# danielbrathwaite/OpenGL-Path-Tracing

Hardware: AMD Instinct MI355X
Metric: Mrays/sec + ms/frame @1920×1080, 8 bounces, 1/2/4/8 MI355X (higher is better)
Workload: dtype f32

## Files before the change

opengl-path-tracing_amd/csrc/pt_pool.h:

```cpp
#pragma once

#include <stdint.h>

#include "pt_math.h"

namespace ptpool {

constexpr int kLanes = 64;
constexpr int kMaxPaths = 128;
constexpr int kRecDwords = 20;
constexpr int kChunks = kRecDwords / 4;

enum : int { kChunkO = 0, kChunkD = 1, kChunkInc = 2, kChunkCol = 3, kChunkItem = 4 };

PT_HD int quad_of(int c, int i, int P) { return c * P + i; }
PT_HD int list_bytes(int P) { return (P + 15) & ~15; }
PT_HD int wave_bytes(int P) { return P * kRecDwords * 4 + list_bytes(P); }

constexpr uint32_t kNoItem = 0xffffffffu;
PT_HD bool pack_ok(int width, int rows_local, int n_frames, int max_bounce, int n_slots, int n_spheres) {
    return width >= 1 && width <= 65535 && rows_local >= 0 && rows_local <= 65535 && n_frames >= 1 &&
           n_frames <= 65535 && max_bounce >= 0 && max_bounce <= 65533 && n_slots >= 0 && n_slots <= 65533 &&
           n_spheres == 1 && (long long)n_frames * (long long)(max_bounce + 2) < (1ll << 31);
}
PT_HD uint32_t pack_xy(int lx, int crow) { return (uint32_t)lx | ((uint32_t)crow << 16); }
PT_HD int xy_lx(uint32_t v) { return (int)(v & 0xffffu); }
PT_HD int xy_crow(uint32_t v) { return (int)(v >> 16); }
PT_HD uint32_t pack_k(int k, int kend) { return (uint32_t)k | ((uint32_t)kend << 16); }
PT_HD int k_k(uint32_t v) { return (int)(v & 0xffffu); }
PT_HD int k_kend(uint32_t v) { return (int)(v >> 16); }
PT_HD uint32_t pack_hit(int hprim, int bounce) { return (uint32_t)(hprim + 2) | ((uint32_t)(bounce + 1) << 16); }
PT_HD int hit_hprim(uint32_t v) { return (int)(v & 0xffffu) - 2; }
PT_HD int hit_bounce(uint32_t v) { return (int)(v >> 16) - 1; }
PT_HD uint32_t with_hprim(uint32_t v, int hprim) { return (v & 0xffff0000u) | (uint32_t)(hprim + 2); }
PT_HD uint32_t pack_cost(uint32_t pcost, bool report) { return pcost | (report ? 0x80000000u : 0u); }
PT_HD uint32_t cost_of(uint32_t v) { return v & 0x7fffffffu; }
PT_HD bool cost_report(uint32_t v) { return (v >> 31) != 0u; }

enum : int { kShade = 0, kLeaf = 1 };
struct Lists { int nS, nL; };

PT_HD int choose(const Lists& l) { return l.nS >= l.nL ? kShade : kLeaf; }
PT_HD int take(const Lists& l, int phase) {
    const int n = phase == kShade ? l.nS : l.nL;
    return n < kLanes ? n : kLanes;
}
PT_HD int pop_index(const Lists& l, int phase, int n, int lane, int P) {
    return phase == kShade ? l.nS - n + lane : P - l.nL + lane;
}
PT_HD void drop(Lists& l, int phase, int n) {
    if (phase == kShade) l.nS -= n; else l.nL -= n;
}
PT_HD int push_index(const Lists& l, int phase, int rank, int P) {
    return phase == kShade ? l.nS + rank : P - 1 - l.nL - rank;
}
PT_HD void grow(Lists& l, int phase, int n) {
    if (phase == kShade) l.nS += n; else l.nL += n;
}

PT_HD size_t block_bytes(int P, int waves, size_t scene_bytes) {
    return ((scene_bytes + 15) & ~(size_t)15) + (size_t)waves * (size_t)wave_bytes(P);
}

}
```

opengl-path-tracing_amd/csrc/pt_render_pool.h:

```cpp
#ifndef PT_POOL_SWEEP_DEPTH
#define PT_POOL_SWEEP_DEPTH 2
#endif
#ifndef PT_POOL_SWEEP_LDS
#define PT_POOL_SWEEP_LDS 1
#endif
#ifndef PT_POOL_SWEEP_SIGNED
#define PT_POOL_SWEEP_SIGNED 1
#endif
#define PT_POOL_SIGNED_ON (PT_POOL_SWEEP_SIGNED && PT_POOL_SWEEP_LDS && PT_POOL_SWEEP_DEPTH > 0)
namespace {

__device__ __forceinline__ void pool_cold_walk(const KParams& p, const SceneView& S, f3 o, f3 d, float& t, int& hprim) {
    int w = 0;
    while (w >= 0) {
        const float4 lo = p.sc.nodes[2 * w], hi = p.sc.nodes[2 * w + 1];
        const int a = __float_as_int(hi.z), b = __float_as_int(hi.w);
        if (!slab(lo, hi, o, d, t)) { w = b; continue; }
        if (a >= 0) { w = a; continue; }
        const int q = (~a) >> 2;
        const int s0 = 2 * __float_as_int(p.sweep_tab[2 * q + 1].w);
        const bool cop = __float_as_int(tri_quad<true>(S, s0 + 1, 1).w) != 0;
        const float4 nda = tri_quad<true>(S, s0, 0);
        const float4 ndb = cop ? nda : tri_quad<true>(S, s0 + 1, 0);
        const float ta = tri_plane(nda, o, d);
        const float tb = cop ? ta : tri_plane(ndb, o, d);
        bool oka = false, okb = false, ca = false, cb = false;
        if (win_open(ta, t)) oka = tri_edges_at<true, false>(S, s0, mk(nda.x, nda.y, nda.z), o + d * ta, false, 0.0f, ca);
        if (win_closed(tb, t)) okb = tri_edges_at<true, false>(S, s0 + 1, mk(ndb.x, ndb.y, ndb.z), o + d * tb, false, 0.0f, cb);
        const float h1 = oka ? ta : -1.0f, h2 = okb ? tb : -1.0f;
        const LeafChoice lc = leaf_choice(h1, h2, t);
        if (lc.c1 | lc.c2) {
            t = lc.c1 ? h1 : h2;
            hprim = s0 + (lc.c1 ? 0 : 1);
        }
        w = b;
    }
}

__device__ __forceinline__ void pool_pass_fence() {
    __builtin_amdgcn_fence(__ATOMIC_RELEASE, "wavefront");
    __builtin_amdgcn_wave_barrier();
    __builtin_amdgcn_fence(__ATOMIC_ACQUIRE, "wavefront");
}

template <int NT, int P, int MINW>
__global__ __launch_bounds__(NT, MINW) void k_render_pool(KParams p) {
    static_assert(P >= 64 && P <= ptpool::kMaxPaths && P % 4 == 0, "one-byte list entries in a 16-byte padded array");
    using namespace ptpool;
    const LaunchFacts<true, true> F{p};
    const const_v4f* const sweep_tab = (const const_v4f*)(size_t)p.sweep_tab;
    (void)sweep_tab;
    resolve_frames(p);
    extern __shared__ float4 lds[];
    const int T = p.n_slots, nt = 4 * T, nm = 3 * p.n_mats, ns = 2, nb = ptc::kSignedQuads * p.n_sweep;
    stage_tris_chain_order(lds, p, T, NT);
    for (int i = threadIdx.x; i < nm; i += NT) lds[nt + i] = p.sc.mats[i];
    for (int i = threadIdx.x; i < ns; i += NT) lds[nt + nm + i] = p.sc.spheres[i];
#if PT_POOL_SIGNED_ON
    for (int leaf = threadIdx.x; leaf < p.n_sweep; leaf += NT) {
        const float4 a = p.sweep_tab[2 * leaf], b = p.sweep_tab[2 * leaf + 1];
        for (int axis = 0; axis < ptc::kSignedQuads; axis++) {
            float q[4];
            ptc::sweep_signed_quad(a, b, axis, q);
            lds[nt + nm + ns + ptc::kSignedQuads * leaf + axis] = make_float4(q[0], q[1], q[2], q[3]);
        }
    }
#else
    for (int i = threadIdx.x; i < 2 * p.n_sweep; i += NT) lds[nt + nm + ns + i] = p.sweep_tab[i];
#endif
    const int scene_q = nt + nm + ns + nb;
    const int lane = (int)(threadIdx.x & 63u);
    float4* const pool = lds + scene_q + (int)(threadIdx.x >> 6) * (wave_bytes(P) / 16);
    unsigned char* const list = (unsigned char*)(pool + kChunks * P);
    for (int i = lane; i < P; i += kLanes) {
        pool[quad_of(kChunkO, i, P)] = make_float4(0, 0, 0, -1.0f);
        pool[quad_of(kChunkD, i, P)] = make_float4(0, 0, 1, 0);
        pool[quad_of(kChunkInc, i, P)] = make_float4(0, 0, 0, __uint_as_float(pack_hit(-1, -1)));
        pool[quad_of(kChunkCol, i, P)] = make_float4(1, 1, 1, 0);
        pool[quad_of(kChunkItem, i, P)] = make_float4(__uint_as_float(kNoItem), 0, 0, 0);
        list[i] = (unsigned char)i;
    }
    __syncthreads();
    SceneView S;
    S.nodes = nullptr;
    S.tris = lds;
    S.mats = lds + nt;
    S.spheres = lds + nt + nm;
    const float4* const boxes = lds + nt + nm + ns;
    const float2* const signed_pairs = (const float2*)boxes;
    (void)signed_pairs;
    S.np = 0;
    S.tp = T;
    S.cm[0] = p.cons_m[0], S.cm[1] = p.cons_m[1], S.cm[2] = p.cons_m[2];
    S.ws[0] = p.win_slack[0], S.ws[1] = p.win_slack[1], S.ws[2] = p.win_slack[2];
    S.clo = ptc::kWindowLo;
    const f3 cpos = mk(p.cam[0], p.cam[1], p.cam[2]), cfwd = mk(p.cam[3], p.cam[4], p.cam[5]);
    const f3 cright = mk(p.cam[6], p.cam[7], p.cam[8]), cup = mk(p.cam[9], p.cam[10], p.cam[11]);
    const int tiles_x = (p.W + 7) >> 3;
    const unsigned n_groups = (unsigned)((p.n_frames + p.group - 1) / p.group);
    const unsigned total_ids = p.queue_tiles * n_groups * 64u;
    unsigned qnext = 0, qend = 0;
    Lists L = {P, 0};
    while (L.nS + L.nL > 0) {
        const int phase = choose(L), n = take(L, phase);
        const bool on = lane < n;
        int idx = 0;
        if (on) idx = list[pop_index(L, phase, n, lane, P)];
        drop(L, phase, n);
        bool to_shade = false, to_leaf = false;
        if (phase == kShade) {
            const float4 c0 = pool[quad_of(kChunkO, idx, P)], c1 = pool[quad_of(kChunkD, idx, P)];
            const float4 c2 = pool[quad_of(kChunkInc, idx, P)], c3 = pool[quad_of(kChunkCol, idx, P)];
            const float4 c4 = pool[quad_of(kChunkItem, idx, P)];
            f3 o = mk(c0.x, c0.y, c0.z), d = mk(c1.x, c1.y, c1.z), inc = mk(c2.x, c2.y, c2.z), col = mk(c3.x, c3.y, c3.z);
            float t = c0.w;
            unsigned bi = __float_as_uint(c1.w);
            int hprim = hit_hprim(__float_as_uint(c2.w)), bounce = hit_bounce(__float_as_uint(c2.w));
            uint32_t state = __float_as_uint(c3.w);
            unsigned xy = __float_as_uint(c4.x);
            int aidx = __float_as_int(c4.y);
            int k = k_k(__float_as_uint(c4.z)), kend = k_kend(__float_as_uint(c4.z));
            unsigned pcost = cost_of(__float_as_uint(c4.w));
            bool report = cost_report(__float_as_uint(c4.w));
            bool retired = false;
            if (on && !(t < 0.0f)) {
                const bool hit = hprim != -1;
                pcost++;
                f3 rgb;
                const bool finished = shade_segment<true>(F, p, S, hit, hprim, t, o, d, inc, col, state, bounce, rgb);
                if (finished) {
                    bounce = -1;
                    const f3 px = (mk(0, 0, 0) + rgb) / 1.0f;
                    nt_store3(p.rgb + 3 * ((size_t)k * (size_t)(p.rows_local * p.W) + (size_t)aidx), px);
                    k++;
                }
                t = -1.0f;
            }
            if (on & (bounce < 0) & (xy != kNoItem) & (k >= kend)) {
                if (report) atomicAdd(&p.tile_cost[(xy_crow(xy) >> 3) * tiles_x + (xy_lx(xy) >> 3)], pcost);
                xy = kNoItem;
            }
            const bool want = on && xy == kNoItem;
            const unsigned long long m = __ballot(want);
            if (m) {
                const QueueIds qi = queue_ids<true>(p, want, m, qnext, qend);
                const unsigned id = qi.id;
                qnext = qi.qnext, qend = qi.qend;
                if (want) {
                    if (id >= total_ids) {
                        retired = true;
                    } else {
                        const unsigned item = id >> 6, w = id & 63u;
                        const unsigned tile = p.grp_magic ? __umulhi(item, p.grp_magic) : item;
                        const int g = (int)(item - tile * n_groups);
                        const unsigned pk = p.tile_perm[tile];
                        const int tx = (int)(pk & 0xffffu), ty = (int)(pk >> 16);
                        const int cx = tx * 8 + (int)(w & 7u);
                        const int crow = ty * 8 + (int)(w >> 3);
                        if ((cx < p.W) & (crow < p.rows_local)) {
                            xy = pack_xy(cx, crow);
                            aidx = crow * p.W + cx;
                            report = (w & 0x1bu) == 0u;
                            pcost = 0;
                            k = g * p.group;
                            kend = min(k + p.group, p.n_frames);
                            bounce = -1;
                        }
                    }
                }
            }
            if (on && xy != kNoItem) {
                const int lx = xy_lx(xy), y = p.row0 + xy_crow(xy) * p.row_stride;
                if (bounce < 0) camera_ray(F, p, cpos, cfwd, cright, cup, lx, y, k, 0, state, o, d, inc, col, bounce);
                const bool fast_seg = seg_in_guard(F, o, d);
                const f3 rd = fast_seg ? mk(pt::rcp_fast(d.x), pt::rcp_fast(d.y), pt::rcp_fast(d.z)) : mk(0, 0, 0);
                t = __builtin_huge_valf();
                hprim = -1;
                {
                    const float ht = sphere_t(S, 0, o, d);
                    if (win_open(ht, t)) {
                        t = ht;
                        hprim = -2;
                    }
                }
                const bool walk = !ray_has_nan(o, d);
#if PT_POOL_SIGNED_ON
                const unsigned cand = sweep_candidates_signed<PT_POOL_SWEEP_DEPTH>(p, S, signed_pairs, walk & fast_seg, o, rd, t);
#elif PT_POOL_SWEEP_DEPTH > 0 && PT_POOL_SWEEP_LDS
                const unsigned cand = sweep_candidates<PT_POOL_SWEEP_DEPTH>(p, S, boxes, walk & fast_seg, o, rd, t);
#else
                const unsigned cand = sweep_candidates<PT_POOL_SWEEP_DEPTH>(p, S, sweep_tab, walk & fast_seg, o, rd, t);
#endif
                const bool cold = walk & !fast_seg;
                if (__any(cold)) {
                    if (cold) pool_cold_walk(p, S, o, d, t, hprim);
                }
                bi = cand;
                to_leaf = cand != 0u;
            }
            to_shade = on & !retired & !to_leaf;
            if (on) {
                pool[quad_of(kChunkO, idx, P)] = make_float4(o.x, o.y, o.z, t);
                pool[quad_of(kChunkD, idx, P)] = make_float4(d.x, d.y, d.z, __uint_as_float(bi));
                pool[quad_of(kChunkInc, idx, P)] = make_float4(inc.x, inc.y, inc.z, __uint_as_float(pack_hit(hprim, bounce)));
                pool[quad_of(kChunkCol, idx, P)] = make_float4(col.x, col.y, col.z, __uint_as_float(state));
                pool[quad_of(kChunkItem, idx, P)] = make_float4(__uint_as_float(xy), __int_as_float(aidx),
                                                                __uint_as_float(pack_k(k, kend)),
                                                                __uint_as_float(pack_cost(pcost, report)));
            }
        } else {
            const float4 c0 = pool[quad_of(kChunkO, idx, P)], c1 = pool[quad_of(kChunkD, idx, P)];
            float* const hw = (float*)&pool[quad_of(kChunkInc, idx, P)] + 3;
            const unsigned hb = __float_as_uint(*hw);
            const f3 o = mk(c0.x, c0.y, c0.z), d = mk(c1.x, c1.y, c1.z);
            float t = c0.w;
            unsigned bi = __float_as_uint(c1.w);
            const bool at = on;
            int s0 = 0, lp = 0;
            bool cop = false;
            float4 nd0 = make_float4(0, 0, 0, 0);
            if (at) {
                lp = __ffs((int)bi) - 1;
                s0 = 2 * lp;
                cop = __float_as_int(tri_quad<true>(S, s0 + 1, 1).w) != 0;
                nd0 = tri_quad<true>(S, s0, 0);
            }
            float h1 = -1.0f, h2 = -1.0f;
            bool ca = false, cb = false;
            leaf_pair_tests<true, false>(S, at, s0, nd0, cop, o, d, t, p.compact_max, h1, h2, false, ca, cb);
            bool c1h = false, c2h = false;
            if (at) {
                const LeafChoice lc = leaf_choice(h1, h2, t);
                c1h = lc.c1, c2h = lc.c2;
            }
            const bool chk = at & (c1h | c2h);
            if (__any(chk)) {
                if (chk) {
                    const f3 rd = mk(pt::rcp_fast(d.x), pt::rcp_fast(d.y), pt::rcp_fast(d.z));
#if PT_POOL_SIGNED_ON
                    const float2 bx = signed_pairs[ptc::kSignedPairs * lp], by = signed_pairs[ptc::kSignedPairs * lp + 2];
                    const float2 bz = signed_pairs[ptc::kSignedPairs * lp + 4];
                    if (!slab_fast(make_float4(bx.x, bx.y, by.x, by.y), make_float4(bz.x, bz.y, 0, 0), o, d, rd, t)) c1h = c2h = false;
#else
                    if (!slab_fast(boxes[2 * lp], boxes[2 * lp + 1], o, d, rd, t)) c1h = c2h = false;
#endif
                }
            }
            if (at) {
                int hprim = hit_hprim(hb);
                if (c1h | c2h) {
                    t = c1h ? h1 : h2;
                    hprim = s0 + (c1h ? 0 : 1);
                }
                bi &= bi - 1u;
                to_leaf = bi != 0u;
                to_shade = bi == 0u;
                ((float*)&pool[quad_of(kChunkO, idx, P)])[3] = t;
                ((float*)&pool[quad_of(kChunkD, idx, P)])[3] = __uint_as_float(bi);
                *hw = __uint_as_float(with_hprim(hb, hprim));
            }
        }
        const unsigned long long mS = __ballot(to_shade), mL = __ballot(to_leaf);
        if (to_shade) list[push_index(L, kShade, rank_in(mS), P)] = (unsigned char)idx;
        if (to_leaf) list[push_index(L, kLeaf, rank_in(mL), P)] = (unsigned char)idx;
        grow(L, kShade, __popcll(mS));
        grow(L, kLeaf, __popcll(mL));
        pool_pass_fence();
    }
}

}
```

Measured before the change: 38700.

## Store ray origin/direction in list-position slots and write hprim as a half-word

The hot ray fields (origin, direction, t, candidate mask) now live in slots indexed by the list position instead of the path index. Each lane in a pass therefore reads a contiguous slot, and the fields are rewritten at the push position when the path is re-queued. The leaf phase also stores only the 16-bit hprim half with a direct write, instead of a read-modify-write of the whole Inc word. This is meant to cut LDS bank conflicts and scattered accesses in the wavefront pool. In exchange, every re-queued path pays an extra 32-byte write per pass, and the scheme relies on the in-pass ordering of reads before pushes.

```diff
diff --git a/opengl-path-tracing_amd/csrc/pt_pool.h b/opengl-path-tracing_amd/csrc/pt_pool.h
--- a/opengl-path-tracing_amd/csrc/pt_pool.h
+++ b/opengl-path-tracing_amd/csrc/pt_pool.h
@@ -14,6 +14,9 @@
 enum : int { kChunkO = 0, kChunkD = 1, kChunkInc = 2, kChunkCol = 3, kChunkItem = 4 };
 
 PT_HD int quad_of(int c, int i, int P) { return c * P + i; }
+PT_HD int cold_quad(int c, int i, int P) { return quad_of(c, i, P); }
+PT_HD int hot_quad(int c, int e, int P) { return quad_of(c, e, P); }
+PT_HD int hprim_half_byte(int i, int P) { return 16 * cold_quad(kChunkInc, i, P) + 12; }
 PT_HD int list_bytes(int P) { return (P + 15) & ~15; }
 PT_HD int wave_bytes(int P) { return P * kRecDwords * 4 + list_bytes(P); }
 
@@ -33,6 +36,7 @@
 PT_HD int hit_hprim(uint32_t v) { return (int)(v & 0xffffu) - 2; }
 PT_HD int hit_bounce(uint32_t v) { return (int)(v >> 16) - 1; }
 PT_HD uint32_t with_hprim(uint32_t v, int hprim) { return (v & 0xffff0000u) | (uint32_t)(hprim + 2); }
+PT_HD uint16_t hprim_half(int hprim) { return (uint16_t)(hprim + 2); }
 PT_HD uint32_t pack_cost(uint32_t pcost, bool report) { return pcost | (report ? 0x80000000u : 0u); }
 PT_HD uint32_t cost_of(uint32_t v) { return v & 0x7fffffffu; }
 PT_HD bool cost_report(uint32_t v) { return (v >> 31) != 0u; }
diff --git a/opengl-path-tracing_amd/csrc/pt_render_pool.h b/opengl-path-tracing_amd/csrc/pt_render_pool.h
--- a/opengl-path-tracing_amd/csrc/pt_render_pool.h
+++ b/opengl-path-tracing_amd/csrc/pt_render_pool.h
@@ -8,6 +8,12 @@
 #define PT_POOL_SWEEP_SIGNED 1
 #endif
 #define PT_POOL_SIGNED_ON (PT_POOL_SWEEP_SIGNED && PT_POOL_SWEEP_LDS && PT_POOL_SWEEP_DEPTH > 0)
+#ifndef PT_POOL_HOT_SLOTS
+#define PT_POOL_HOT_SLOTS 1
+#endif
+#ifndef PT_POOL_HPRIM_HALF
+#define PT_POOL_HPRIM_HALF 1
+#endif
 namespace {
 
 __device__ __forceinline__ void pool_cold_walk(const KParams& p, const SceneView& S, f3 o, f3 d, float& t, int& hprim) {
@@ -104,17 +110,28 @@
     while (L.nS + L.nL > 0) {
         const int phase = choose(L), n = take(L, phase);
         const bool on = lane < n;
+        const int e = on ? pop_index(L, phase, n, lane, P) : 0;
+#if PT_POOL_HOT_SLOTS
+        const int idx = list[e];
+        const int hs = e;
+#else
         int idx = 0;
-        if (on) idx = list[pop_index(L, phase, n, lane, P)];
+        if (on) idx = list[e];
+        const int hs = idx;
+#endif
         drop(L, phase, n);
         bool to_shade = false, to_leaf = false;
+        f3 o = mk(0, 0, 0), d = mk(0, 0, 0);
+        float t = 0.0f;
+        unsigned bi = 0u;
         if (phase == kShade) {
-            const float4 c0 = pool[quad_of(kChunkO, idx, P)], c1 = pool[quad_of(kChunkD, idx, P)];
-            const float4 c2 = pool[quad_of(kChunkInc, idx, P)], c3 = pool[quad_of(kChunkCol, idx, P)];
-            const float4 c4 = pool[quad_of(kChunkItem, idx, P)];
-            f3 o = mk(c0.x, c0.y, c0.z), d = mk(c1.x, c1.y, c1.z), inc = mk(c2.x, c2.y, c2.z), col = mk(c3.x, c3.y, c3.z);
-            float t = c0.w;
-            unsigned bi = __float_as_uint(c1.w);
+            const float4 c0 = pool[hot_quad(kChunkO, hs, P)], c1 = pool[hot_quad(kChunkD, hs, P)];
+            const float4 c2 = pool[cold_quad(kChunkInc, idx, P)], c3 = pool[cold_quad(kChunkCol, idx, P)];
+            const float4 c4 = pool[cold_quad(kChunkItem, idx, P)];
+            f3 inc = mk(c2.x, c2.y, c2.z), col = mk(c3.x, c3.y, c3.z);
+            o = mk(c0.x, c0.y, c0.z), d = mk(c1.x, c1.y, c1.z);
+            t = c0.w;
+            bi = __float_as_uint(c1.w);
             int hprim = hit_hprim(__float_as_uint(c2.w)), bounce = hit_bounce(__float_as_uint(c2.w));
             uint32_t state = __float_as_uint(c3.w);
             unsigned xy = __float_as_uint(c4.x);
@@ -200,21 +217,25 @@
             }
             to_shade = on & !retired & !to_leaf;
             if (on) {
+#if !PT_POOL_HOT_SLOTS
                 pool[quad_of(kChunkO, idx, P)] = make_float4(o.x, o.y, o.z, t);
                 pool[quad_of(kChunkD, idx, P)] = make_float4(d.x, d.y, d.z, __uint_as_float(bi));
-                pool[quad_of(kChunkInc, idx, P)] = make_float4(inc.x, inc.y, inc.z, __uint_as_float(pack_hit(hprim, bounce)));
-                pool[quad_of(kChunkCol, idx, P)] = make_float4(col.x, col.y, col.z, __uint_as_float(state));
-                pool[quad_of(kChunkItem, idx, P)] = make_float4(__uint_as_float(xy), __int_as_float(aidx),
-                                                                __uint_as_float(pack_k(k, kend)),
-                                                                __uint_as_float(pack_cost(pcost, report)));
+#endif
+                pool[cold_quad(kChunkInc, idx, P)] = make_float4(inc.x, inc.y, inc.z, __uint_as_float(pack_hit(hprim, bounce)));
+                pool[cold_quad(kChunkCol, idx, P)] = make_float4(col.x, col.y, col.z, __uint_as_float(state));
+                pool[cold_quad(kChunkItem, idx, P)] = make_float4(__uint_as_float(xy), __int_as_float(aidx),
+                                                                 __uint_as_float(pack_k(k, kend)),
+                                                                 __uint_as_float(pack_cost(pcost, report)));
             }
         } else {
-            const float4 c0 = pool[quad_of(kChunkO, idx, P)], c1 = pool[quad_of(kChunkD, idx, P)];
-            float* const hw = (float*)&pool[quad_of(kChunkInc, idx, P)] + 3;
+            const float4 c0 = pool[hot_quad(kChunkO, hs, P)], c1 = pool[hot_quad(kChunkD, hs, P)];
+#if !PT_POOL_HPRIM_HALF
+            float* const hw = (float*)&pool[cold_quad(kChunkInc, idx, P)] + 3;
             const unsigned hb = __float_as_uint(*hw);
-            const f3 o = mk(c0.x, c0.y, c0.z), d = mk(c1.x, c1.y, c1.z);
-            float t = c0.w;
-            unsigned bi = __float_as_uint(c1.w);
+#endif
+            o = mk(c0.x, c0.y, c0.z), d = mk(c1.x, c1.y, c1.z);
+            t = c0.w;
+            bi = __float_as_uint(c1.w);
             const bool at = on;
             int s0 = 0, lp = 0;
             bool cop = false;
@@ -247,22 +268,40 @@
                 }
             }
             if (at) {
+#if PT_POOL_HPRIM_HALF
+                if (c1h | c2h) {
+                    t = c1h ? h1 : h2;
+                    *(uint16_t*)((char*)pool + hprim_half_byte(idx, P)) = hprim_half(s0 + (c1h ? 0 : 1));
+                }
+#else
                 int hprim = hit_hprim(hb);
                 if (c1h | c2h) {
                     t = c1h ? h1 : h2;
                     hprim = s0 + (c1h ? 0 : 1);
                 }
+                *hw = __uint_as_float(with_hprim(hb, hprim));
+#endif
                 bi &= bi - 1u;
                 to_leaf = bi != 0u;
                 to_shade = bi == 0u;
+#if !PT_POOL_HOT_SLOTS
                 ((float*)&pool[quad_of(kChunkO, idx, P)])[3] = t;
                 ((float*)&pool[quad_of(kChunkD, idx, P)])[3] = __uint_as_float(bi);
-                *hw = __uint_as_float(with_hprim(hb, hprim));
+#endif
             }
         }
         const unsigned long long mS = __ballot(to_shade), mL = __ballot(to_leaf);
+#if PT_POOL_HOT_SLOTS
+        if (to_shade | to_leaf) {
+            const int pe = to_shade ? push_index(L, kShade, rank_in(mS), P) : push_index(L, kLeaf, rank_in(mL), P);
+            list[pe] = (unsigned char)idx;
+            pool[hot_quad(kChunkO, pe, P)] = make_float4(o.x, o.y, o.z, t);
+            pool[hot_quad(kChunkD, pe, P)] = make_float4(d.x, d.y, d.z, __uint_as_float(bi));
+        }
+#else
         if (to_shade) list[push_index(L, kShade, rank_in(mS), P)] = (unsigned char)idx;
         if (to_leaf) list[push_index(L, kLeaf, rank_in(mL), P)] = (unsigned char)idx;
+#endif
         grow(L, kShade, __popcll(mS));
         grow(L, kLeaf, __popcll(mL));
         pool_pass_fence();
```

Result: no change. 38990 (median of 6 runs) (+0.7%).
